# 1adrianb/binary-networks-pytorch

Hardware: AMD Instinct MI355X
Metric: images/sec binary ResNet-18 224x224 forward (higher is better)
Workload: dtype int1 xnor-popcount on the integer ALU (19 binary convs: two bit planes, v_bitop3_b32 + v_bcnt_u32_b32, int32 accumulation) + fp32 epilogues (alpha, BN, residual) + stem conv with fp32 operands split into fp16 hi+lo on v_mfma_f32_16x16x32_f16, fp32 accumulation (3e-7 relative; not IEEE fp32 — the exa

## Files before the change

binary-networks-pytorch_amd/bnn_amd/fastpath.py:

```python
from __future__ import annotations

import os
import threading
import warnings
import weakref
from dataclasses import dataclass
from typing import Optional

import torch
import torch.nn as nn

from . import hipops, native

_stats_lock = threading.Lock()
_stats = {"conv2d": 0, "conv1d": 0, "linear": 0, "weight_packs": 0, "conv2d_train": 0, "cell_op": 0, "cell": 0,
          "cell_op_train": 0, "reduce_train": 0, "linear_train": 0, "conv2d_real": 0, "conv2d_real_train": 0,
          "linear_real": 0, "linear_real_train": 0, "fconv": 0}

REAL_WEIGHTS = os.environ.get("BNN_AMD_REAL_WEIGHTS", "0") == "1"

MFMA_CONV = os.environ.get("BNN_AMD_MFMA_CONV", "1")
MFMA_CONV_SHAPES = {
    (128, 128, 28, 1, False): ((51.9, 37.8), (58.6, 45.2)),
    (128, 256, 28, 2, False): ((30.3, 26.2),),
    (256, 256, 14, 1, False): ((54.9, 33.4), (56.9, 38.9)),
    (256, 512, 14, 2, False): ((33.6, 23.8),),
    (512, 512, 7, 1, False): ((60.6, 32.0), (63.3, 39.2)),
}


def mfma_conv_admitted(C: int, O: int, H: int, stride: int, fold: bool) -> bool:
    if MFMA_CONV == "0":
        return False
    return MFMA_CONV == "all" or (C, O, H, stride, fold) in MFMA_CONV_SHAPES


MFMA_FOLD = os.environ.get("BNN_AMD_MFMA_FOLD", "1")
MFMA_FOLD_SHAPES = {
    (128, 128, 28, 64): (71.0, 61.2),
    (256, 256, 14, 128): (66.0, 50.3),
    (512, 512, 7, 256): (71.8, 45.3),
}


def mfma_fold_admitted(C: int, O: int, H: int, sc_C: int) -> bool:
    if MFMA_CONV == "0" or MFMA_FOLD == "0":
        return False
    return MFMA_FOLD == "all" or (C, O, H, sc_C) in MFMA_FOLD_SHAPES


FCONV_DECLINED_SHAPES = {
}


def fconv_admitted(C: int, H: int, W: int, stride: int) -> bool:
    return (C, H, W, stride) not in FCONV_DECLINED_SHAPES


def stats() -> dict:
    with _stats_lock:
        return dict(_stats)


def _bump(key: str) -> None:
    with _stats_lock:
        _stats[key] += 1


def strict_weights() -> bool:
    return os.environ.get("BNN_AMD_STRICT_WEIGHTS", "0") == "1"


@dataclass
class Plan:
    center: bool
    compute_alpha: bool
    scale: Optional[torch.Tensor]
    ste: bool = True


@dataclass
class RealPlan:
    scale: Optional[torch.Tensor]
    ste: bool = True


_HOOK_MODULES = ("bnn_amd.ops", "bnn_amd.bconfig", "bnn.ops", "bnn.bconfig")


def _is(obj, name: str) -> bool:
    t = type(obj)
    return t.__name__ == name and t.__module__ in _HOOK_MODULES


def _input_hook(pre) -> Optional[bool]:
    if _is(pre, "BasicInputBinarizer"):
        return True
    advanced = (_is(pre, "AdvancedInputBinarizer") and getattr(pre, "derivative_funct", None) is torch.tanh
                and isinstance(getattr(pre, "t", None), (int, float)) and pre.t > 0)
    return False if advanced else None


def _post_scale(post, out_channels: int):
    if _is(post, "Identity"):
        return True, None
    if _is(post, "BasicScaleBinarizer") and post.alpha.numel() == out_channels \
            and post.alpha.dim() >= 2 and post.alpha.shape[1] == out_channels:
        return True, post.alpha
    return False, None


def _recognise(layer: nn.Module, out_channels: int) -> Optional[Plan]:
    wpre = layer.weight_pre_process
    basic = _input_hook(layer.activation_pre_process)
    if basic is None or not _is(wpre, "XNORWeightBinarizer"):
        return None
    ok, scale = _post_scale(layer.activation_post_process, out_channels)
    if not ok:
        return None
    return Plan(bool(wpre.center_weights), bool(wpre.compute_alpha), scale, ste=basic)


def _recognise_real(layer: nn.Module, out_channels: int) -> Optional[RealPlan]:
    wpre = layer.weight_pre_process
    basic = _input_hook(layer.activation_pre_process)
    if basic is None:
        return None
    if not (type(wpre) is nn.Identity or _is(wpre, "Identity")) or wpre._forward_hooks or wpre._forward_pre_hooks:
        return None
    ok, scale = _post_scale(layer.activation_post_process, out_channels)
    if not ok:
        return None
    return RealPlan(scale, ste=basic)


def _eligible(layer: nn.Module, x: torch.Tensor, plan: Plan) -> bool:
    w = layer.weight
    if not (x.is_cuda and w.is_cuda and x.device == w.device):
        return False
    if x.dtype != w.dtype or x.dtype not in (torch.float32, torch.float16):
        return False
    if torch.is_grad_enabled():
        needs = x.requires_grad or w.requires_grad
        needs = needs or (layer.bias is not None and layer.bias.requires_grad)
        needs = needs or (plan.scale is not None and plan.scale.requires_grad)
        if needs:
            return False
    return True


def _eligible_train(layer: nn.Module, x: torch.Tensor) -> bool:
    from . import training
    w = layer.weight
    return (training.ENABLED and torch.is_grad_enabled() and x.is_cuda and w.is_cuda and x.device == w.device
            and x.dtype == torch.float32 and w.dtype == torch.float32)


def _numeric_padding(layer) -> bool:
    return not isinstance(layer.padding, str) and layer.padding_mode == "zeros" and layer.groups == 1


def _grouped_numeric_padding(layer) -> bool:
    return not isinstance(layer.padding, str) and layer.padding_mode == "zeros" and layer.groups > 1


def plan_conv2d(layer, x: torch.Tensor) -> Optional[Plan]:
    if x.dim() != 4 or not (_numeric_padding(layer) or _grouped_numeric_padding(layer)):
        return None
    plan = _recognise(layer, layer.out_channels)
    return plan if plan is not None and _eligible(layer, x, plan) else None


def plan_conv2d_train(layer, x: torch.Tensor) -> Optional[Plan]:
    from . import training
    if x.dim() != 4 or not (_numeric_padding(layer) or (training.GROUPED and _grouped_numeric_padding(layer))):
        return None
    plan = _recognise(layer, layer.out_channels)
    return plan if plan is not None and plan.ste and _eligible_train(layer, x) else None


def _real_applies(layer, x: torch.Tensor) -> Optional[RealPlan]:
    if not REAL_WEIGHTS or x.dim() != 4 or not _numeric_padding(layer) or torch.is_autocast_enabled():
        return None
    if x.dtype != torch.float32 or layer.weight.dtype != torch.float32:
        return None
    plan = _recognise_real(layer, layer.out_channels)
    if plan is None or not hipops.sconv_supported(x.shape, layer.weight.shape, layer.stride, layer.padding, layer.dilation):
        return None
    return plan


def plan_conv2d_real(layer, x: torch.Tensor) -> Optional[RealPlan]:
    plan = _real_applies(layer, x)
    return plan if plan is not None and _eligible(layer, x, plan) else None


def plan_conv2d_real_train(layer, x: torch.Tensor) -> Optional[RealPlan]:
    plan = _real_applies(layer, x)
    return plan if plan is not None and plan.ste and _eligible_train(layer, x) else None


def _real_linear_applies(layer, x: torch.Tensor) -> Optional[RealPlan]:
    if not REAL_WEIGHTS or x.dim() < 1 or torch.is_autocast_enabled():
        return None
    if x.dtype != torch.float32 or layer.weight.dtype != torch.float32:
        return None
    return _recognise_real(layer, layer.out_features)


def plan_linear_real(layer, x: torch.Tensor) -> Optional[RealPlan]:
    plan = _real_linear_applies(layer, x)
    return plan if plan is not None and _eligible(layer, x, plan) else None


def plan_linear_real_train(layer, x: torch.Tensor) -> Optional[RealPlan]:
    plan = _real_linear_applies(layer, x)
    return plan if plan is not None and plan.ste and _eligible_train(layer, x) else None


def plan_conv1d(layer, x: torch.Tensor) -> Optional[Plan]:
    if x.dim() != 3 or not (_numeric_padding(layer) or _grouped_numeric_padding(layer)):
        return None
    plan = _recognise(layer, layer.out_channels)
    return plan if plan is not None and _eligible(layer, x, plan) else None


def plan_linear(layer, x: torch.Tensor) -> Optional[Plan]:
    if x.dim() < 1:
        return None
    plan = _recognise(layer, layer.out_features)
    return plan if plan is not None and _eligible(layer, x, plan) else None


def plan_linear_train(layer, x: torch.Tensor) -> Optional[Plan]:
    from . import training
    if not training.LINEAR or x.dim() < 1 or torch.is_autocast_enabled():
        return None
    plan = _recognise(layer, layer.out_features)
    if plan is None or not plan.ste or not _eligible_train(layer, x):
        return None
    return plan if training._no_hooks(layer.weight_pre_process, backward=False) else None


def packed_weight(layer, plan: Plan, sync: bool = True, fresh: bool = False) -> hipops.PackedWeight:
    if strict_weights():
        sync, fresh = True, True
    master = layer.__dict__.get("_bnn_master")
    if master is not None:
        return _replica_packed_weight(layer, master, plan, fresh)
    w = layer.weight
    groups = getattr(layer, "groups", 1)
    key = (w.data_ptr(), w._version, str(w.device), tuple(w.shape), plan.center, plan.compute_alpha, groups)
    cached = layer.__dict__.get("_bnn_packed")
    sync = sync or cached is None
    if cached is not None and cached[1].zero_probe is not None and (sync or fresh or cached[0] != key):
        pw = cached[1]
        if pw.zero_found_later():
            layer.__dict__["_bnn_zero_seen"] = True
            warnings.warn("bnn_amd: a binary weight is exactly 0 (sign(0) == 0); a forward that ran before this "
                          "was known treated it as -1.  This layer now takes the zero-aware kernels.",
                          RuntimeWarning)
            cached = None
        else:
            pw.zero_probe = None
    if cached is not None and cached[0] == key and not fresh:
        return cached[1]
    sync = sync or layer.__dict__.get("_bnn_zero_seen", False)
    pw = _pack(w, plan, groups, sync)
    if pw.has_zero:
        layer.__dict__["_bnn_zero_seen"] = True
    layer.__dict__["_bnn_packed"] = (key, pw)
    _bump("weight_packs")
    return pw


def _pack(w: torch.Tensor, plan: Plan, groups: int, sync: bool) -> hipops.PackedWeight:
    if groups != 1:
        return hipops.pack_weight_grouped(w, groups, plan.center, plan.compute_alpha, sync=sync)
    return hipops.pack_weight(w, plan.center, plan.compute_alpha, sync=sync)


def _replica_packed_weight(layer, master, plan: Plan, fresh: bool = False) -> hipops.PackedWeight:
    mw = master.weight
    w = layer.weight
    groups = getattr(layer, "groups", 1)
    key = (mw.data_ptr(), mw._version, tuple(mw.shape), plan.center, plan.compute_alpha, groups)
    cache = master.__dict__.setdefault("_bnn_packed_replicas", {})
    dev = str(w.device)
    hit = cache.get(dev)
    if hit is not None and hit[0] == key and not fresh:
        return hit[1]
    pw = _pack(w, plan, groups, sync=True)
    cache[dev] = (key, pw)
    _bump("weight_packs")
    return pw


BLOCK_KEY, OP_KEY, CELL_KEY = TIER_KEYS = ("_bnn_auto_block", "_bnn_auto_op", "_bnn_auto_cell")


WATCH_KEY = "_bnn_watchers"


class _Watchers:

    def __init__(self) -> None:
        self.refs = weakref.WeakSet()

    def __deepcopy__(self, memo) -> "_Watchers":
        return _Watchers()

    def __reduce__(self):
        return (_Watchers, ())


def watch(model: nn.Module, executor) -> None:
    model.__dict__.setdefault(WATCH_KEY, _Watchers()).refs.add(executor)


def drop_executor(m: nn.Module) -> None:
    for key in TIER_KEYS:
        m.__dict__.pop(key, None)


def invalidate(module: nn.Module, executors: bool = True) -> int:
    n = 0
    for m in module.modules():
        if m.__dict__.pop("_bnn_packed", None) is not None:
            n += 1
        if m.__dict__.pop(REAL_KEY, None) is not None:
            n += 1
        m.__dict__.pop("_bnn_packed_replicas", None)
        if executors:
            drop_executor(m)
            for ex in tuple(getattr(m.__dict__.get(WATCH_KEY), "refs", ())):
                ex.mark_stale()
    from .tails import drop_derived
    drop_derived(module)
    return n


def _f32(t: Optional[torch.Tensor]) -> Optional[torch.Tensor]:
    return t if t is None or t.dtype == torch.float32 else t.detach().float()


def conv2d(layer, x: torch.Tensor, plan: Plan) -> torch.Tensor:
    native.require()
    pw = packed_weight(layer, plan)
    if layer.groups != 1:
        out = hipops.bconv2d_grouped(hipops.pack_act(x), pw, _f32(layer.bias), _f32(plan.scale), layer.stride,
                                     layer.padding, layer.dilation)
        _bump("conv2d")
        return out.to(x.dtype)
    out = hipops.bconv2d_direct(x, pw, _f32(layer.bias), _f32(plan.scale), layer.stride, layer.padding,
                                layer.dilation)
    _bump("conv2d")
    return out.to(x.dtype)


def conv2d_train(layer, x: torch.Tensor, plan: Plan) -> torch.Tensor:
    from . import training
    native.require()
    out = training.conv2d_train(layer, x, plan, packed_weight(layer, plan, sync=False, fresh=True))
    _bump("conv2d_train")
    return out


REAL_KEY = "_bnn_packed_real"


def real_packed_weight(layer) -> hipops.SconvWeight:
    w = layer.weight
    key = (w.data_ptr(), w._version, str(w.device), tuple(w.shape), "sconv")
    cached = layer.__dict__.get(REAL_KEY)
    if cached is not None and cached[0] == key and not strict_weights():
        return cached[1]
    pw = hipops.slinear_pack_weight(w) if w.dim() == 2 else hipops.sconv_pack_weight(w)
    layer.__dict__[REAL_KEY] = (key, pw)
    _bump("weight_packs")
    return pw


def conv2d_real(layer, x: torch.Tensor, plan: RealPlan) -> torch.Tensor:
    native.require()
    out = hipops.sconv2d(x, real_packed_weight(layer), layer.bias, plan.scale, layer.stride, layer.padding)
    _bump("conv2d_real")
    return out


def conv2d_real_train(layer, x: torch.Tensor, plan: RealPlan) -> torch.Tensor:
    from . import training
    native.require()
    out = training.sconv2d_train(layer, x, plan)
    _bump("conv2d_real_train")
    return out


def linear_real(layer, x: torch.Tensor, plan: RealPlan) -> torch.Tensor:
    native.require()
    scale = None if plan.scale is None else plan.scale.reshape(-1)
    out = hipops.slinear(x, real_packed_weight(layer), layer.bias, scale)
    _bump("linear_real")
    return out


def linear_real_train(layer, x: torch.Tensor, plan: RealPlan) -> torch.Tensor:
    from . import training
    native.require()
    out = training.slinear_train(layer, x, plan)
    _bump("linear_real_train")
    return out


def conv1d(layer, x: torch.Tensor, plan: Plan) -> torch.Tensor:
    native.require()
    pw = packed_weight(layer, plan)
    if layer.groups != 1:
        out = hipops.bconv2d_grouped(hipops.pack_act(x.unsqueeze(2)), pw, _f32(layer.bias), _f32(plan.scale),
                                     (1, layer.stride[0]), (0, layer.padding[0]), (1, layer.dilation[0]))
        _bump("conv1d")
        return out.squeeze(2).to(x.dtype)
    out = hipops.bconv2d_direct(x.unsqueeze(2), pw, _f32(layer.bias), _f32(plan.scale), (1, layer.stride[0]),
                                (0, layer.padding[0]), (1, layer.dilation[0]))
    _bump("conv1d")
    return out.squeeze(2).to(x.dtype)


def linear(layer, x: torch.Tensor, plan: Plan) -> torch.Tensor:
    native.require()
    pw = packed_weight(layer, plan)
    out = hipops.linear(x, pw, _f32(layer.bias), _f32(plan.scale))
    _bump("linear")
    return out.to(x.dtype)


def linear_train(layer, x: torch.Tensor, plan: Plan) -> torch.Tensor:
    from . import training
    native.require()
    out = training.linear_train(layer, x, plan, packed_weight(layer, plan, sync=False, fresh=True))
    _bump("linear_train")
    return out
```

binary-networks-pytorch_amd/csrc/bconv_mfma.hip:

```cpp
#include "bconv_core.h"

namespace bnn {

namespace {

using i32x4 = __attribute__((ext_vector_type(4))) int;

constexpr int kMfmaThreads = 256;
constexpr int kAccStride = 68;
constexpr int kAccBytes = 4 * 32 * kAccStride * 4;
constexpr int kMaxLds = 64 * 1024;
constexpr int kPatchSlots = 4;
constexpr int kParkStride = 72;
constexpr int kParkBytes = 4 * 64 * kParkStride * 2;
constexpr int kMaxLdsFold = 80 * 1024;

struct MfmaGeo {
  int tp;
  int groups;
  int ihw;
  int patch_cap;
  int nn;
  int n_in;
  uint32_t m_ihw;
  int s_ihw;
  int park_off;
};

struct ShortcutArgs8 {
  const uint32_t* P;
  const int8_t* W8;
  const float* alpha;
  const float* a;
  const float* b;
};

__device__ __forceinline__ uint32_t spread4(uint32_t word, int sh) {
  return __umul24((word >> sh) & 15u, 0x00204081u) & 0x01010101u;
}
__device__ __forceinline__ uint32_t expand4(uint32_t pw, uint32_t mw, int sh, bool nn) {
  const uint32_t p = spread4(pw, sh);
  if (nn) return p;
  return p | (spread4(mw, sh) * 0xFFu);
}

__device__ __forceinline__ int centre_of(const Geo& g, const MfmaGeo& mg, int q, int* oy, int* ox) {
  const int hw = g.Ho * g.Wo;
  const int n = (int)fast_div((uint32_t)q, g.m_hw, g.s_hw);
  const int r = q - n * hw;
  *oy = (int)fast_div((uint32_t)r, g.m_wo, g.s_wo);
  *ox = r - *oy * g.Wo;
  return n * mg.ihw + *oy * g.sh * g.Wd + *ox * g.sw;
}

template <int EP, bool DS = false>
__global__ __launch_bounds__(kMfmaThreads) void bconv_mfma_kernel(const uint32_t* __restrict__ P,
                                                                  const uint32_t* __restrict__ M,
                                                                  const int8_t* __restrict__ W8, BNN_EPI_PARAMS,
                                                                  const Geo g, const MfmaGeo mg,
                                                                  const uint32_t* __restrict__ dsP,
                                                                  const int8_t* __restrict__ dsW8,
                                                                  const float* __restrict__ ds_alpha,
                                                                  const float* __restrict__ ds_a,
                                                                  const float* __restrict__ ds_b) {
  static_assert(!DS || EP == EP_OUT, "the fold belongs to BN + residual + ReLU -> fp32 + planes");
  BNN_EPI_INIT;
  [[maybe_unused]] const ShortcutArgs8 sc{dsP, dsW8, ds_alpha, ds_a, ds_b};
  extern __shared__ __attribute__((aligned(16))) unsigned char lds[];
  const int tid = threadIdx.x, lane = tid & 63;
  const int wave = __builtin_amdgcn_readfirstlane(tid >> 6);
  const int lrow = lane & 15, lgrp = lane >> 4;
  const int pwaves = mg.tp >> 6;
  const int wave_pix = (wave % pwaves) * 64;
  const int wave_ch = (wave / pwaves) * 64;
  const int q0 = blockIdx.x * mg.tp;
  const int o_wave = blockIdx.y * (64 * (4 / pwaves)) + wave_ch;

  int ty, tx;
  const int c_first = centre_of(g, mg, q0, &ty, &tx);
  const int c_last = centre_of(g, mg, min(q0 + mg.tp, g.npix) - 1, &ty, &tx);
  const int l_lo = max(c_first - g.Wd - 1, 0);
  const int patch_len = min(min(c_last + g.Wd + 1, mg.n_in - 1) - l_lo + 1, mg.patch_cap);
  const int zero_idx = mg.patch_cap;

  int base[4];
  uint32_t okm[4];
#pragma unroll
  for (int pt = 0; pt < 4; ++pt) {
    const int q = min(q0 + wave_pix + 16 * pt + lrow, g.npix - 1);
    int oy, ox;
    base[pt] = centre_of(g, mg, q, &oy, &ox) - l_lo;
    uint32_t m = 0u;
#pragma unroll
    for (int t = 0; t < 9; ++t) {
      const int iy = oy * g.sh - 1 + t / 3, ix = ox * g.sw - 1 + t % 3;
      const bool ok = (unsigned)iy < (unsigned)g.H && (unsigned)ix < (unsigned)g.Wd;
      m |= (ok ? 1u : 0u) << t;
    }
    okm[pt] = m;
  }

  i32x4 acc[4][4];
#pragma unroll
  for (int ct = 0; ct < 4; ++ct)
#pragma unroll
    for (int pt = 0; pt < 4; ++pt) acc[ct][pt] = i32x4{0, 0, 0, 0};

  if (tid < 4) reinterpret_cast<uint4*>(lds + (size_t)zero_idx * 64)[tid] = uint4{0u, 0u, 0u, 0u};

  const bool nn = mg.nn != 0;
  const uint2* P2 = reinterpret_cast<const uint2*>(P);
  const uint2* M2 = reinterpret_cast<const uint2*>(M);
  const int8_t* wbase = W8 + (size_t)(o_wave >> 6) * mg.groups * (9 * 4096) + lane * 16;

  const int ksteps = mg.groups * 9;
  auto a_load = [&](i32x4 (&dst)[4], int k) {
    const int8_t* src = wbase + (size_t)min(k, ksteps - 1) * 4096;
#pragma unroll
    for (int ct = 0; ct < 4; ++ct) dst[ct] = *reinterpret_cast<const i32x4*>(src + ct * 1024);
  };
  auto b_frag = [&](int pt, int t) -> i32x4 {
    const int off = (t / 3 - 1) * g.Wd + (t % 3 - 1);
    const int idx = ((okm[pt] >> t) & 1u) ? min(base[pt] + off, zero_idx) : zero_idx;
    return *reinterpret_cast<const i32x4*>(lds + (size_t)idx * 64 + lgrp * 16);
  };
  unsigned wi0[kPatchSlots];
  uint2 pv[kPatchSlots], mv[kPatchSlots];
#pragma unroll
  for (int sl = 0; sl < kPatchSlots; ++sl) {
    const int L = l_lo + min(tid + sl * kMfmaThreads, patch_len - 1);
    const int n = (int)fast_div((uint32_t)L, mg.m_ihw, mg.s_ihw);
    wi0[sl] = (unsigned)(n * mg.groups * mg.ihw + (L - n * mg.ihw));
    pv[sl] = uint2{0u, 0u};
    mv[sl] = uint2{0u, 0u};
  }
  auto request = [&](int gi) {
#pragma unroll
    for (int sl = 0; sl < kPatchSlots; ++sl)
      if (sl * kMfmaThreads < patch_len) {
        pv[sl] = P2[wi0[sl] + (unsigned)(gi * mg.ihw)];
        if (!nn) mv[sl] = M2[wi0[sl] + (unsigned)(gi * mg.ihw)];
      }
  };
  auto expand = [&]() {
#pragma unroll
    for (int sl = 0; sl < kPatchSlots; ++sl) {
      const int i = tid + sl * kMfmaThreads;
      if (i < patch_len) {
        uint4* dst = reinterpret_cast<uint4*>(lds + (size_t)i * 64);
#pragma unroll
        for (int h = 0; h < 4; ++h) {
          const uint32_t pw = h < 2 ? pv[sl].x : pv[sl].y, mw = h < 2 ? mv[sl].x : mv[sl].y;
          const int s0 = 16 * (h & 1);
          dst[h] = uint4{expand4(pw, mw, s0, nn), expand4(pw, mw, s0 + 4, nn), expand4(pw, mw, s0 + 8, nn),
                         expand4(pw, mw, s0 + 12, nn)};
        }
      }
    }
  };

  request(0);
  i32x4 a_buf[3][4];
  if constexpr (DS) {
    const int sg = g.ds_cw >> 1;
    uint2 scw[4];
    {
      const int q = min(q0 + tid, g.npix - 1), hw = g.Ho * g.Wo;
      const int n = (int)fast_div((uint32_t)q, g.m_hw, g.s_hw), r = q - n * hw;
      const int oy = (int)fast_div((uint32_t)r, g.m_wo, g.s_wo), ox = r - oy * g.Wo;
      const uint2* S2 = reinterpret_cast<const uint2*>(sc.P);
      if (g.ds_w > 0) {
        const unsigned shw = (unsigned)(g.ds_h * g.ds_w);
        const int y0 = 2 * oy, x0 = 2 * ox;
        const bool x1 = x0 + 1 < g.ds_w, y1 = y0 + 1 < g.ds_h;
        const unsigned b0 = (unsigned)n * (unsigned)sg * shw + (unsigned)(y0 * g.ds_w + x0);
        static_for<4>([&](auto GI) {
          constexpr int gi = GI;
          uint2 v{0u, 0u};
          if (gi < sg) {
            const unsigned b = b0 + (unsigned)gi * shw;
            v = S2[b];
            const uint2 a = S2[x1 ? b + 1 : b], c = S2[y1 ? b + (unsigned)g.ds_w : b],
                        e = S2[(x1 && y1) ? b + (unsigned)g.ds_w + 1 : b];
            v.x |= a.x | c.x | e.x;
            v.y |= a.y | c.y | e.y;
          }
          scw[gi] = v;
        });
      } else {
        const unsigned b0 = (unsigned)n * (unsigned)sg * (unsigned)hw + (unsigned)r;
        static_for<4>([&](auto GI) {
          constexpr int gi = GI;
          scw[gi] = gi < sg ? S2[b0 + (unsigned)(gi * hw)] : uint2{0u, 0u};
        });
      }
    }
    const int8_t* sbase = sc.W8 + (size_t)(o_wave >> 6) * sg * 4096 + lane * 16;
    auto sa_load = [&](i32x4 (&dst)[4], int k) {
      const int8_t* src = sbase + (size_t)min(k, sg - 1) * 4096;
#pragma unroll
      for (int ct = 0; ct < 4; ++ct) dst[ct] = *reinterpret_cast<const i32x4*>(src + ct * 1024);
    };
    sa_load(a_buf[0], 0);
    sa_load(a_buf[1], 1);
    static_for<4>([&](auto K) {
      constexpr int k = K;
      if (k < sg) {
        if (k > 0) __syncthreads();
        if (tid < mg.tp) {
          uint4* dst = reinterpret_cast<uint4*>(lds + (size_t)tid * 64);
#pragma unroll
          for (int h = 0; h < 4; ++h) {
            const uint32_t pw = h < 2 ? scw[k].x : scw[k].y;
            const int s0 = 16 * (h & 1);
            dst[h] = uint4{expand4(pw, 0u, s0, true), expand4(pw, 0u, s0 + 4, true), expand4(pw, 0u, s0 + 8, true),
                           expand4(pw, 0u, s0 + 12, true)};
          }
        }
        __syncthreads();
        sa_load(a_buf[(k + 2) % 3], k + 2);
        i32x4 b_sc[4];
#pragma unroll
        for (int pt = 0; pt < 4; ++pt)
          b_sc[pt] = *reinterpret_cast<const i32x4*>(lds + (size_t)(wave_pix + 16 * pt + lrow) * 64 + lgrp * 16);
        __builtin_amdgcn_sched_barrier(0);
#pragma unroll
        for (int ct = 0; ct < 4; ++ct)
#pragma unroll
          for (int pt = 0; pt < 4; ++pt)
            acc[ct][pt] = __builtin_amdgcn_mfma_i32_16x16x64_i8(a_buf[k % 3][ct], b_sc[pt], acc[ct][pt], 0, 0, 0);
        __builtin_amdgcn_sched_barrier(0);
      }
    });
  }
  a_load(a_buf[0], 0);
  a_load(a_buf[1], 1);
  if constexpr (DS) {
    short* park = reinterpret_cast<short*>(lds + mg.park_off) + wave * (64 * kParkStride);
#pragma unroll
    for (int ct = 0; ct < 4; ++ct)
#pragma unroll
      for (int pt = 0; pt < 4; ++pt) {
        const i32x4 v = acc[ct][pt];
        *reinterpret_cast<uint2*>(park + (16 * pt + lrow) * kParkStride + 16 * ct + 4 * lgrp) =
            uint2{((uint32_t)v[0] & 0xFFFFu) | ((uint32_t)v[1] << 16), ((uint32_t)v[2] & 0xFFFFu) | ((uint32_t)v[3] << 16)};
        acc[ct][pt] = i32x4{0, 0, 0, 0};
      }
  }
#pragma unroll 1
  for (int gi = 0; gi < mg.groups; ++gi) {
    __syncthreads();
    expand();
    __syncthreads();
    if (gi + 1 < mg.groups) request(gi + 1);
    i32x4 b_cur[4];
#pragma unroll
    for (int pt = 0; pt < 4; ++pt) b_cur[pt] = b_frag(pt, 0);
#pragma unroll
    for (int t = 0; t < 9; ++t) {
      i32x4 b_nxt[4];
      a_load(a_buf[(t + 2) % 3], gi * 9 + t + 2);
      if (t < 8) {
#pragma unroll
        for (int pt = 0; pt < 4; ++pt) b_nxt[pt] = b_frag(pt, t + 1);
      }
      __builtin_amdgcn_sched_barrier(0);
#pragma unroll
      for (int ct = 0; ct < 4; ++ct)
#pragma unroll
        for (int pt = 0; pt < 4; ++pt)
          acc[ct][pt] = __builtin_amdgcn_mfma_i32_16x16x64_i8(a_buf[t % 3][ct], b_cur[pt], acc[ct][pt], 0, 0, 0);
      __builtin_amdgcn_sched_barrier(0);
      if (t < 8) {
#pragma unroll
        for (int pt = 0; pt < 4; ++pt) b_cur[pt] = b_nxt[pt];
      }
    }
  }

  const Pix px = decode_pixel<true>(g, q0 + wave_pix + lane);
  int* tbuf = reinterpret_cast<int*>(lds) + wave * (32 * kAccStride);
#pragma unroll
  for (int h = 0; h < 2; ++h) {
    const int o0 = o_wave + 32 * h;
    float resv[32];
    if constexpr (DS) {
      using f2 = __attribute__((ext_vector_type(2))) float;
      const uint4* pr = reinterpret_cast<const uint4*>(reinterpret_cast<const short*>(lds + mg.park_off) +
                                                       wave * (64 * kParkStride) + lane * kParkStride + 32 * h);
      uint32_t w[16];
#pragma unroll
      for (int i = 0; i < 4; ++i) {
        const uint4 v = pr[i];
        w[4 * i] = v.x; w[4 * i + 1] = v.y; w[4 * i + 2] = v.z; w[4 * i + 3] = v.w;
      }
#pragma unroll
      for (int j = 0; j < 32; j += 2) {
        const int o = o0 + j;
        const f2 d = f2{(float)((int)(w[j >> 1] << 16) >> 16), (float)((int)w[j >> 1] >> 16)};
        const f2 t = __builtin_elementwise_fma(f2{sc.alpha[o], sc.alpha[o + 1]}, d, f2{0.0f, 0.0f});
        const f2 r = __builtin_elementwise_fma(t, f2{sc.a[o], sc.a[o + 1]}, f2{sc.b[o], sc.b[o + 1]});
        resv[j] = r.x;
        resv[j + 1] = r.y;
      }
    } else {
      prefetch_residual<32, EP, true>(g, px, o0, epi, resv);
    }
    __syncthreads();
#pragma unroll
    for (int c2 = 0; c2 < 2; ++c2)
#pragma unroll
      for (int pt = 0; pt < 4; ++pt)
#pragma unroll
        for (int r = 0; r < 4; ++r)
          tbuf[(16 * c2 + 4 * lgrp + r) * kAccStride + 16 * pt + lrow] = acc[2 * h + c2][pt][r];
    __syncthreads();
    int dot[32];
#pragma unroll
    for (int j = 0; j < 32; ++j) dot[j] = tbuf[j * kAccStride + lane];
    uint32_t pbits = 0u, mbits = 0u;
    epilogue<32, EP, true>(g, px, o0, dot, resv, epi, pbits, mbits, 0, 1.0f, 0.0f);
    uint32_t xorw = 0u;
    if constexpr (EP == EP_MIDT) xorw = (uint32_t)epi.thr[kThrStride * o0 + 1];
    store_packed(g, px, o0 >> 5, pbits, mbits, epi, true, xorw);
  }
}

__global__ __launch_bounds__(256) void pack_weight_i8_kernel(const uint32_t* __restrict__ wbits,
                                                             const uint32_t* __restrict__ wnz, int O, int taps,
                                                             int cw32, int cwc, uint32_t* __restrict__ w8) {
  const int groups = cw32 >> 1, nchunk = cw32 / cwc, per_o = taps * cwc;
  const size_t total = (size_t)O * groups * taps * 16;
  const size_t d = (size_t)blockIdx.x * 256 + threadIdx.x;
  if (d >= total) return;
  const int e4 = (int)(d & 3), lane = (int)((d >> 2) & 63), ct = (int)((d >> 8) & 3);
  size_t rest = d >> 10;
  const int t = (int)(rest % taps);
  rest /= taps;
  const int gi = (int)(rest % groups), ob64 = (int)(rest / groups);
  const int o = 64 * ob64 + 16 * ct + (lane & 15);
  const int c0 = 64 * gi + 16 * (lane >> 4) + 4 * e4;
  const int cw_abs = c0 >> 5, ch = cw_abs / cwc, cw = cw_abs - ch * cwc;
  const size_t wi = ((size_t)((o >> 5) * nchunk + ch) * kOCB + (o & 31)) * per_o + t * cwc + cw;
  const uint32_t b = wbits[wi] >> (c0 & 31), z = wnz ? wnz[wi] >> (c0 & 31) : 15u;
  uint32_t v = 0u;
#pragma unroll
  for (int k = 0; k < 4; ++k) {
    const uint32_t byte = ((z >> k) & 1u) ? (((b >> k) & 1u) ? 0x01u : 0xFFu) : 0u;
    v |= byte << (8 * k);
  }
  w8[d] = v;
}

long long centre_span(const ConvP& p, int tp) {
  const long long s = p.sw, k = tp - 1, hw = (long long)p.Ho * p.Wo;
  const long long row_extra = (long long)p.sh * p.Wd - (long long)p.Wo * s;
  const long long img_extra = (long long)p.H * p.Wd - (long long)p.Ho * p.sh * p.Wd;
  return k * s + (k + p.Wo - 1) / p.Wo * (row_extra > 0 ? row_extra : 0) + (k + hw - 1) / hw * (img_extra > 0 ? img_extra : 0);
}

size_t lds_bytes_of(int patch_cap) {
  const size_t patch = (size_t)(patch_cap + 1) * 64;
  return patch > (size_t)kAccBytes ? patch : (size_t)kAccBytes;
}

int choose_tile(const ConvP& p, int* patch_cap, size_t park = 0) {
  const size_t lds_max = park ? (size_t)kMaxLdsFold : (size_t)kMaxLds;
  const int order[2] = {(p.O % 128 == 0 && p.C >= 128) ? 128 : 256, (p.O % 128 == 0 && p.C >= 128) ? 256 : 128};
  for (int tp : order) {
    if (tp == 128 && p.O % 128 != 0) continue;
    const long long cap = centre_span(p, tp) + 2LL * p.Wd + 3;
    if (cap <= kPatchSlots * kMfmaThreads && lds_bytes_of((int)cap) + park <= lds_max) {
      *patch_cap = (int)cap;
      return tp;
    }
  }
  return 0;
}

template <int EP>
void launch_ep(const ConvP& p, const Geo& g, const MfmaGeo& mg, const void* w8, dim3 grid, size_t ldsb, hipStream_t s) {
  hipLaunchKernelGGL((bconv_mfma_kernel<EP>), grid, dim3(kMfmaThreads), ldsb, s, p.P, p.M,
                     static_cast<const int8_t*>(w8), BNN_EPI_ACTUALS, g, mg, static_cast<const uint32_t*>(nullptr),
                     static_cast<const int8_t*>(nullptr), static_cast<const float*>(nullptr),
                     static_cast<const float*>(nullptr), static_cast<const float*>(nullptr));
}

}

size_t weight_i8_bytes(int O, int C, int KH, int KW) {
  if (O <= 0 || C <= 0 || KH != 3 || KW != 3 || O % 64 != 0 || C % 64 != 0) return 0;
  return (size_t)O * (size_t)C * 9;
}

int launch_pack_weight_i8(const uint32_t* wbits, const uint32_t* wnz, const bnn_hip_wlayout& L, int O, void* w8,
                          hipStream_t s) {
  const size_t dwords = (size_t)O * (L.cw32 >> 1) * L.taps * 16;
  hipLaunchKernelGGL(pack_weight_i8_kernel, dim3((unsigned)((dwords + 255) / 256)), dim3(256), 0, s, wbits, wnz, O, L.taps,
                     L.cw32, L.cwc, static_cast<uint32_t*>(w8));
  return hipGetLastError() == hipSuccess ? BNN_HIP_OK : BNN_HIP_ERR_LAUNCH;
}

size_t shortcut_weight_i8_bytes(int O, int C) {
  if (O <= 0 || O % 64 != 0 || (C != 64 && C != 128 && C != 256)) return 0;
  return (size_t)O * (size_t)C;
}

int launch_pack_shortcut_weight_i8(const uint32_t* wbits, int O, int C, void* w8, hipStream_t s) {
  const int cw32 = C / 32;
  const size_t dwords = (size_t)O * (cw32 >> 1) * 16;
  hipLaunchKernelGGL(pack_weight_i8_kernel, dim3((unsigned)((dwords + 255) / 256)), dim3(256), 0, s, wbits,
                     static_cast<const uint32_t*>(nullptr), O, 1, cw32, cw32, static_cast<uint32_t*>(w8));
  return hipGetLastError() == hipSuccess ? BNN_HIP_OK : BNN_HIP_ERR_LAUNCH;
}

namespace {
bool mfma_dense_rule(const ConvP& p, int flags, size_t park) {
  if (flags & BNN_HIP_FLAG_FORCE_GENERIC) return false;
  if (p.KH != 3 || p.KW != 3 || p.ph != 1 || p.pw != 1 || p.dh != 1 || p.dw != 1) return false;
  if (p.sh != p.sw || (p.sh != 1 && p.sh != 2)) return false;
  if (p.C % 64 != 0 || p.O % 64 != 0 || !small_indices(p)) return false;
  if (p.raw || p.prelu || p.pack_a || p.pack_b || p.eflags != 0) return false;
  if (p.c_off != 0 || p.c_tot != p.O) return false;
  if ((long long)p.N * p.H * p.Wd >= (1ll << 30)) return false;
  int cap = 0;
  return choose_tile(p, &cap, park) != 0;
}
}

bool mfma_conv_applies(const ConvP& p, int flags) { return !p.ds_P && mfma_dense_rule(p, flags, 0); }

bool mfma_fold_applies(const ConvP& p, int flags) {
  if (!p.ds_P || p.res || p.thr) return false;
  if (!(flags & BNN_HIP_FLAG_ACT_NONNEG) || (flags & BNN_HIP_FLAG_WEIGHT_ZEROS)) return false;
  if (shortcut_weight_i8_bytes(p.O, p.ds_C) == 0) return false;
  if (make_geo(p).flags != kFlagsOut) return false;
  return mfma_dense_rule(p, flags, (size_t)kParkBytes);
}

namespace {
MfmaGeo make_mfma_geo(const ConvP& p, int flags, int tp, int cap) {
  MfmaGeo mg;
  mg.tp = tp;
  mg.groups = p.C / 64;
  mg.ihw = p.H * p.Wd;
  mg.patch_cap = cap;
  mg.nn = (flags & BNN_HIP_FLAG_ACT_NONNEG) ? 1 : 0;
  mg.n_in = p.N * p.H * p.Wd;
  div_magic((uint32_t)mg.ihw, mg.m_ihw, mg.s_ihw);
  mg.park_off = (int)lds_bytes_of(cap);
  return mg;
}
}

int launch_bconv_mfma_fold(const ConvP& p, int flags, const void* w8, const void* sc_w8, hipStream_t s) {
  int cap = 0;
  const int tp = choose_tile(p, &cap, (size_t)kParkBytes);
  if (!mfma_fold_applies(p, flags) || tp == 0) return BNN_HIP_ERR_UNSUPPORTED;
  const Geo g = make_geo(p);
  const MfmaGeo mg = make_mfma_geo(p, flags, tp, cap);
  const dim3 grid((unsigned)((p.npix + tp - 1) / tp), (unsigned)(p.O / (tp == 256 ? 64 : 128)));
  const size_t ldsb = lds_bytes_of(cap) + (size_t)kParkBytes;
  auto kern = bconv_mfma_kernel<EP_OUT, true>;
  if (hipFuncSetAttribute(reinterpret_cast<const void*>(kern), hipFuncAttributeMaxDynamicSharedMemorySize,
                          kMaxDynamicLds) != hipSuccess)
    return BNN_HIP_ERR_LAUNCH;
  hipLaunchKernelGGL(kern, grid, dim3(kMfmaThreads), ldsb, s, p.P, p.M, static_cast<const int8_t*>(w8), BNN_EPI_ACTUALS, g,
                     mg, p.ds_P, static_cast<const int8_t*>(sc_w8), p.ds_alpha, p.ds_a, p.ds_b);
  return hipGetLastError() == hipSuccess ? BNN_HIP_OK : BNN_HIP_ERR_LAUNCH;
}

int launch_bconv_mfma(const ConvP& p, int flags, const void* w8, hipStream_t s) {
  int cap = 0;
  const int tp = choose_tile(p, &cap);
  if (!mfma_conv_applies(p, flags) || tp == 0) return BNN_HIP_ERR_UNSUPPORTED;
  const Geo g = make_geo(p);
  const MfmaGeo mg = make_mfma_geo(p, flags, tp, cap);
  const dim3 grid((unsigned)((p.npix + tp - 1) / tp), (unsigned)(p.O / (tp == 256 ? 64 : 128)));
  const size_t ldsb = lds_bytes_of(cap);
  const int f = g.flags;
  const bool fused = (f & (EF_BN | EF_RES | EF_RELU | EF_PACK)) != 0;
  if (f == kFlagsMid && p.thr) launch_ep<EP_MIDT>(p, g, mg, w8, grid, ldsb, s);
  else if (f == kFlagsMid) launch_ep<EP_MID>(p, g, mg, w8, grid, ldsb, s);
  else if (f == kFlagsOut) launch_ep<EP_OUT>(p, g, mg, w8, grid, ldsb, s);
  else if (f == kFlagsOutP) launch_ep<EP_OUTP>(p, g, mg, w8, grid, ldsb, s);
  else if (f == kFlagsLast) launch_ep<EP_LAST>(p, g, mg, w8, grid, ldsb, s);
  else if (fused) launch_ep<EP_RUNTIME>(p, g, mg, w8, grid, ldsb, s);
  else launch_ep<EP_PLAIN>(p, g, mg, w8, grid, ldsb, s);
  return hipGetLastError() == hipSuccess ? BNN_HIP_OK : BNN_HIP_ERR_LAUNCH;
}

}
```

Before: 328,000.

## Reshape MFMA binary conv wave tile to 128 pixels by 32 channels with padded LDS planes

Each wave now covers 128 pixels by 32 output channels instead of 64 by 64. The LDS patch is stored as four separate 16-byte planes, and a virtual zero row is inserted between image rows. Border handling uses precomputed left, centre and right addresses plus a far address clamped to a zero slot, which replaces the per-tap validity mask and index clamp. The aim is to cut LDS address arithmetic and bank conflicts and to change A/B fragment reuse, at the cost of more B fragment loads per wave, more registers, and a larger patch span.

Result: no change. 328,800 (median of 3 runs) (+0.3%).

```diff
diff --git a/binary-networks-pytorch_amd/bnn_amd/fastpath.py b/binary-networks-pytorch_amd/bnn_amd/fastpath.py
--- a/binary-networks-pytorch_amd/bnn_amd/fastpath.py
+++ b/binary-networks-pytorch_amd/bnn_amd/fastpath.py
@@ -21,11 +21,11 @@
 
 MFMA_CONV = os.environ.get("BNN_AMD_MFMA_CONV", "1")
 MFMA_CONV_SHAPES = {
-    (128, 128, 28, 1, False): ((51.9, 37.8), (58.6, 45.2)),
-    (128, 256, 28, 2, False): ((30.3, 26.2),),
-    (256, 256, 14, 1, False): ((54.9, 33.4), (56.9, 38.9)),
-    (256, 512, 14, 2, False): ((33.6, 23.8),),
-    (512, 512, 7, 1, False): ((60.6, 32.0), (63.3, 39.2)),
+    (128, 128, 28, 1, False): ((51.9, 38.0), (58.6, 47.8)),
+    (128, 256, 28, 2, False): ((30.3, 27.8),),
+    (256, 256, 14, 1, False): ((54.9, 34.3), (56.9, 39.7)),
+    (256, 512, 14, 2, False): ((33.6, 23.6),),
+    (512, 512, 7, 1, False): ((60.6, 32.2), (63.3, 41.4)),
 }
 
 
@@ -37,9 +37,9 @@
 
 MFMA_FOLD = os.environ.get("BNN_AMD_MFMA_FOLD", "1")
 MFMA_FOLD_SHAPES = {
-    (128, 128, 28, 64): (71.0, 61.2),
-    (256, 256, 14, 128): (66.0, 50.3),
-    (512, 512, 7, 256): (71.8, 45.3),
+    (128, 128, 28, 64): (71.0, 60.8),
+    (256, 256, 14, 128): (66.0, 47.5),
+    (512, 512, 7, 256): (71.8, 44.8),
 }
 
 
diff --git a/binary-networks-pytorch_amd/csrc/bconv_mfma.hip b/binary-networks-pytorch_amd/csrc/bconv_mfma.hip
--- a/binary-networks-pytorch_amd/csrc/bconv_mfma.hip
+++ b/binary-networks-pytorch_amd/csrc/bconv_mfma.hip
@@ -11,8 +11,11 @@
 constexpr int kAccBytes = 4 * 32 * kAccStride * 4;
 constexpr int kMaxLds = 64 * 1024;
 constexpr int kPatchSlots = 4;
-constexpr int kParkStride = 72;
-constexpr int kParkBytes = 4 * 64 * kParkStride * 2;
+constexpr int kWavePix = 128;
+constexpr int kWaveCh = 32;
+constexpr uint32_t kFarAddr = 0x40000000u;
+constexpr int kParkStride = 36;
+constexpr int kParkBytes = 4 * kWavePix * kParkStride * 2;
 constexpr int kMaxLdsFold = 80 * 1024;
 
 struct MfmaGeo {
@@ -20,10 +23,14 @@
   int groups;
   int ihw;
   int patch_cap;
+  int plane;
   int nn;
-  int n_in;
-  uint32_t m_ihw;
-  int s_ihw;
+  int hp;
+  int n_pad;
+  uint32_t m_w;
+  int s_w;
+  uint32_t m_hp;
+  int s_hp;
   int park_off;
 };
 
@@ -50,7 +57,7 @@
   const int r = q - n * hw;
   *oy = (int)fast_div((uint32_t)r, g.m_wo, g.s_wo);
   *ox = r - *oy * g.Wo;
-  return n * mg.ihw + *oy * g.sh * g.Wd + *ox * g.sw;
+  return (n * mg.hp + *oy * g.sh + 1) * g.Wd + *ox * g.sw;
 }
 
 template <int EP, bool DS = false>
@@ -70,74 +77,73 @@
   const int tid = threadIdx.x, lane = tid & 63;
   const int wave = __builtin_amdgcn_readfirstlane(tid >> 6);
   const int lrow = lane & 15, lgrp = lane >> 4;
-  const int pwaves = mg.tp >> 6;
-  const int wave_pix = (wave % pwaves) * 64;
-  const int wave_ch = (wave / pwaves) * 64;
+  const int pwaves = mg.tp >> 7;
+  const int wave_pix = (wave % pwaves) * kWavePix;
+  const int wave_ch = (wave / pwaves) * kWaveCh;
   const int q0 = blockIdx.x * mg.tp;
-  const int o_wave = blockIdx.y * (64 * (4 / pwaves)) + wave_ch;
+  const int o_wave = blockIdx.y * (kWaveCh * (4 / pwaves)) + wave_ch;
 
   int ty, tx;
   const int c_first = centre_of(g, mg, q0, &ty, &tx);
   const int c_last = centre_of(g, mg, min(q0 + mg.tp, g.npix) - 1, &ty, &tx);
   const int l_lo = max(c_first - g.Wd - 1, 0);
-  const int patch_len = min(min(c_last + g.Wd + 1, mg.n_in - 1) - l_lo + 1, mg.patch_cap);
-  const int zero_idx = mg.patch_cap;
-
-  int base[4];
-  uint32_t okm[4];
-#pragma unroll
-  for (int pt = 0; pt < 4; ++pt) {
+  const int patch_len = min(min(c_last + g.Wd + 1, mg.n_pad - 1) - l_lo + 1, mg.patch_cap);
+  const uint32_t zero_addr = (uint32_t)(3 * mg.plane + mg.patch_cap * 16);
+
+  uint32_t ad_c[8], ad_l[8], ad_r[8];
+#pragma unroll
+  for (int pt = 0; pt < 8; ++pt) {
     const int q = min(q0 + wave_pix + 16 * pt + lrow, g.npix - 1);
     int oy, ox;
-    base[pt] = centre_of(g, mg, q, &oy, &ox) - l_lo;
-    uint32_t m = 0u;
-#pragma unroll
-    for (int t = 0; t < 9; ++t) {
-      const int iy = oy * g.sh - 1 + t / 3, ix = ox * g.sw - 1 + t % 3;
-      const bool ok = (unsigned)iy < (unsigned)g.H && (unsigned)ix < (unsigned)g.Wd;
-      m |= (ok ? 1u : 0u) << t;
-    }
-    okm[pt] = m;
-  }
-
-  i32x4 acc[4][4];
-#pragma unroll
-  for (int ct = 0; ct < 4; ++ct)
-#pragma unroll
-    for (int pt = 0; pt < 4; ++pt) acc[ct][pt] = i32x4{0, 0, 0, 0};
-
-  if (tid < 4) reinterpret_cast<uint4*>(lds + (size_t)zero_idx * 64)[tid] = uint4{0u, 0u, 0u, 0u};
+    const int base = centre_of(g, mg, q, &oy, &ox) - l_lo;
+    const int ix = ox * g.sw;
+    ad_c[pt] = (uint32_t)(base * 16 + lgrp * mg.plane);
+    ad_l[pt] = ix >= 1 ? ad_c[pt] - 16u : kFarAddr;
+    ad_r[pt] = ix + 1 < g.Wd ? ad_c[pt] + 16u : kFarAddr;
+  }
+  const int row_bytes = g.Wd * 16;
+
+  i32x4 acc[2][8];
+#pragma unroll
+  for (int ct = 0; ct < 2; ++ct)
+#pragma unroll
+    for (int pt = 0; pt < 8; ++pt) acc[ct][pt] = i32x4{0, 0, 0, 0};
+
+  if (tid == 0) *reinterpret_cast<uint4*>(lds + zero_addr) = uint4{0u, 0u, 0u, 0u};
 
   const bool nn = mg.nn != 0;
   const uint2* P2 = reinterpret_cast<const uint2*>(P);
   const uint2* M2 = reinterpret_cast<const uint2*>(M);
-  const int8_t* wbase = W8 + (size_t)(o_wave >> 6) * mg.groups * (9 * 4096) + lane * 16;
+  const int8_t* wbase = W8 + (size_t)(o_wave >> 6) * mg.groups * (9 * 4096) + ((o_wave & 63) >> 4) * 1024 + lane * 16;
 
   const int ksteps = mg.groups * 9;
-  auto a_load = [&](i32x4 (&dst)[4], int k) {
+  auto a_load = [&](i32x4 (&dst)[2], int k) {
     const int8_t* src = wbase + (size_t)min(k, ksteps - 1) * 4096;
 #pragma unroll
-    for (int ct = 0; ct < 4; ++ct) dst[ct] = *reinterpret_cast<const i32x4*>(src + ct * 1024);
+    for (int ct = 0; ct < 2; ++ct) dst[ct] = *reinterpret_cast<const i32x4*>(src + ct * 1024);
   };
   auto b_frag = [&](int pt, int t) -> i32x4 {
-    const int off = (t / 3 - 1) * g.Wd + (t % 3 - 1);
-    const int idx = ((okm[pt] >> t) & 1u) ? min(base[pt] + off, zero_idx) : zero_idx;
-    return *reinterpret_cast<const i32x4*>(lds + (size_t)idx * 64 + lgrp * 16);
+    const int dy = t / 3 - 1, dx = t % 3 - 1;
+    const uint32_t off = (uint32_t)(dy * row_bytes);
+    const uint32_t addr = dx == 0 ? ad_c[pt] + off : min((dx < 0 ? ad_l[pt] : ad_r[pt]) + off, zero_addr);
+    return *reinterpret_cast<const i32x4*>(lds + addr);
   };
+  constexpr unsigned kZeroRow = 0xFFFFFFFFu;
   unsigned wi0[kPatchSlots];
   uint2 pv[kPatchSlots], mv[kPatchSlots];
 #pragma unroll
   for (int sl = 0; sl < kPatchSlots; ++sl) {
     const int L = l_lo + min(tid + sl * kMfmaThreads, patch_len - 1);
-    const int n = (int)fast_div((uint32_t)L, mg.m_ihw, mg.s_ihw);
-    wi0[sl] = (unsigned)(n * mg.groups * mg.ihw + (L - n * mg.ihw));
+    const int row = (int)fast_div((uint32_t)L, mg.m_w, mg.s_w), x = L - row * g.Wd;
+    const int n = (int)fast_div((uint32_t)row, mg.m_hp, mg.s_hp), yy = row - n * mg.hp;
+    wi0[sl] = yy == 0 ? kZeroRow : (unsigned)(n * mg.groups * mg.ihw + (yy - 1) * g.Wd + x);
     pv[sl] = uint2{0u, 0u};
     mv[sl] = uint2{0u, 0u};
   }
   auto request = [&](int gi) {
 #pragma unroll
     for (int sl = 0; sl < kPatchSlots; ++sl)
-      if (sl * kMfmaThreads < patch_len) {
+      if (sl * kMfmaThreads < patch_len && wi0[sl] != kZeroRow) {
         pv[sl] = P2[wi0[sl] + (unsigned)(gi * mg.ihw)];
         if (!nn) mv[sl] = M2[wi0[sl] + (unsigned)(gi * mg.ihw)];
       }
@@ -147,20 +153,20 @@
     for (int sl = 0; sl < kPatchSlots; ++sl) {
       const int i = tid + sl * kMfmaThreads;
       if (i < patch_len) {
-        uint4* dst = reinterpret_cast<uint4*>(lds + (size_t)i * 64);
 #pragma unroll
         for (int h = 0; h < 4; ++h) {
           const uint32_t pw = h < 2 ? pv[sl].x : pv[sl].y, mw = h < 2 ? mv[sl].x : mv[sl].y;
           const int s0 = 16 * (h & 1);
-          dst[h] = uint4{expand4(pw, mw, s0, nn), expand4(pw, mw, s0 + 4, nn), expand4(pw, mw, s0 + 8, nn),
-                         expand4(pw, mw, s0 + 12, nn)};
+          *reinterpret_cast<uint4*>(lds + h * mg.plane + i * 16) =
+              uint4{expand4(pw, mw, s0, nn), expand4(pw, mw, s0 + 4, nn), expand4(pw, mw, s0 + 8, nn),
+                    expand4(pw, mw, s0 + 12, nn)};
         }
       }
     }
   };
 
   request(0);
-  i32x4 a_buf[3][4];
+  i32x4 a_buf[3][2];
   if constexpr (DS) {
     const int sg = g.ds_cw >> 1;
     uint2 scw[4];
@@ -195,11 +201,11 @@
         });
       }
     }
-    const int8_t* sbase = sc.W8 + (size_t)(o_wave >> 6) * sg * 4096 + lane * 16;
-    auto sa_load = [&](i32x4 (&dst)[4], int k) {
+    const int8_t* sbase = sc.W8 + (size_t)(o_wave >> 6) * sg * 4096 + ((o_wave & 63) >> 4) * 1024 + lane * 16;
+    auto sa_load = [&](i32x4 (&dst)[2], int k) {
       const int8_t* src = sbase + (size_t)min(k, sg - 1) * 4096;
 #pragma unroll
-      for (int ct = 0; ct < 4; ++ct) dst[ct] = *reinterpret_cast<const i32x4*>(src + ct * 1024);
+      for (int ct = 0; ct < 2; ++ct) dst[ct] = *reinterpret_cast<const i32x4*>(src + ct * 1024);
     };
     sa_load(a_buf[0], 0);
     sa_load(a_buf[1], 1);
@@ -208,26 +214,26 @@
       if (k < sg) {
         if (k > 0) __syncthreads();
         if (tid < mg.tp) {
-          uint4* dst = reinterpret_cast<uint4*>(lds + (size_t)tid * 64);
 #pragma unroll
           for (int h = 0; h < 4; ++h) {
             const uint32_t pw = h < 2 ? scw[k].x : scw[k].y;
             const int s0 = 16 * (h & 1);
-            dst[h] = uint4{expand4(pw, 0u, s0, true), expand4(pw, 0u, s0 + 4, true), expand4(pw, 0u, s0 + 8, true),
-                           expand4(pw, 0u, s0 + 12, true)};
+            *reinterpret_cast<uint4*>(lds + h * mg.plane + tid * 16) =
+                uint4{expand4(pw, 0u, s0, true), expand4(pw, 0u, s0 + 4, true), expand4(pw, 0u, s0 + 8, true),
+                      expand4(pw, 0u, s0 + 12, true)};
           }
         }
         __syncthreads();
         sa_load(a_buf[(k + 2) % 3], k + 2);
-        i32x4 b_sc[4];
-#pragma unroll
-        for (int pt = 0; pt < 4; ++pt)
-          b_sc[pt] = *reinterpret_cast<const i32x4*>(lds + (size_t)(wave_pix + 16 * pt + lrow) * 64 + lgrp * 16);
+        i32x4 b_sc[8];
+#pragma unroll
+        for (int pt = 0; pt < 8; ++pt)
+          b_sc[pt] = *reinterpret_cast<const i32x4*>(lds + lgrp * mg.plane + (wave_pix + 16 * pt + lrow) * 16);
         __builtin_amdgcn_sched_barrier(0);
 #pragma unroll
-        for (int ct = 0; ct < 4; ++ct)
-#pragma unroll
-          for (int pt = 0; pt < 4; ++pt)
+        for (int ct = 0; ct < 2; ++ct)
+#pragma unroll
+          for (int pt = 0; pt < 8; ++pt)
             acc[ct][pt] = __builtin_amdgcn_mfma_i32_16x16x64_i8(a_buf[k % 3][ct], b_sc[pt], acc[ct][pt], 0, 0, 0);
         __builtin_amdgcn_sched_barrier(0);
       }
@@ -236,11 +242,11 @@
   a_load(a_buf[0], 0);
   a_load(a_buf[1], 1);
   if constexpr (DS) {
-    short* park = reinterpret_cast<short*>(lds + mg.park_off) + wave * (64 * kParkStride);
-#pragma unroll
-    for (int ct = 0; ct < 4; ++ct)
-#pragma unroll
-      for (int pt = 0; pt < 4; ++pt) {
+    short* park = reinterpret_cast<short*>(lds + mg.park_off) + wave * (kWavePix * kParkStride);
+#pragma unroll
+    for (int ct = 0; ct < 2; ++ct)
+#pragma unroll
+      for (int pt = 0; pt < 8; ++pt) {
         const i32x4 v = acc[ct][pt];
         *reinterpret_cast<uint2*>(park + (16 * pt + lrow) * kParkStride + 16 * ct + 4 * lgrp) =
             uint2{((uint32_t)v[0] & 0xFFFFu) | ((uint32_t)v[1] << 16), ((uint32_t)v[2] & 0xFFFFu) | ((uint32_t)v[3] << 16)};
@@ -253,46 +259,46 @@
     expand();
     __syncthreads();
     if (gi + 1 < mg.groups) request(gi + 1);
-    i32x4 b_cur[4];
-#pragma unroll
-    for (int pt = 0; pt < 4; ++pt) b_cur[pt] = b_frag(pt, 0);
+    i32x4 b_cur[8];
+#pragma unroll
+    for (int pt = 0; pt < 8; ++pt) b_cur[pt] = b_frag(pt, 0);
 #pragma unroll
     for (int t = 0; t < 9; ++t) {
-      i32x4 b_nxt[4];
+      i32x4 b_nxt[8];
       a_load(a_buf[(t + 2) % 3], gi * 9 + t + 2);
       if (t < 8) {
 #pragma unroll
-        for (int pt = 0; pt < 4; ++pt) b_nxt[pt] = b_frag(pt, t + 1);
+        for (int pt = 0; pt < 8; ++pt) b_nxt[pt] = b_frag(pt, t + 1);
       }
       __builtin_amdgcn_sched_barrier(0);
 #pragma unroll
-      for (int ct = 0; ct < 4; ++ct)
-#pragma unroll
-        for (int pt = 0; pt < 4; ++pt)
+      for (int ct = 0; ct < 2; ++ct)
+#pragma unroll
+        for (int pt = 0; pt < 8; ++pt)
           acc[ct][pt] = __builtin_amdgcn_mfma_i32_16x16x64_i8(a_buf[t % 3][ct], b_cur[pt], acc[ct][pt], 0, 0, 0);
       __builtin_amdgcn_sched_barrier(0);
       if (t < 8) {
 #pragma unroll
-        for (int pt = 0; pt < 4; ++pt) b_cur[pt] = b_nxt[pt];
+        for (int pt = 0; pt < 8; ++pt) b_cur[pt] = b_nxt[pt];
       }
     }
   }
 
-  const Pix px = decode_pixel<true>(g, q0 + wave_pix + lane);
   int* tbuf = reinterpret_cast<int*>(lds) + wave * (32 * kAccStride);
+  const int o0 = o_wave;
 #pragma unroll
   for (int h = 0; h < 2; ++h) {
-    const int o0 = o_wave + 32 * h;
+    const Pix px = decode_pixel<true>(g, q0 + wave_pix + 64 * h + lane);
     float resv[32];
     if constexpr (DS) {
       using f2 = __attribute__((ext_vector_type(2))) float;
-      const uint4* pr = reinterpret_cast<const uint4*>(reinterpret_cast<const short*>(lds + mg.park_off) +
-                                                       wave * (64 * kParkStride) + lane * kParkStride + 32 * h);
+      const uint2* pr = reinterpret_cast<const uint2*>(reinterpret_cast<const short*>(lds + mg.park_off) +
+                                                       wave * (kWavePix * kParkStride) + (64 * h + lane) * kParkStride);
       uint32_t w[16];
 #pragma unroll
-      for (int i = 0; i < 4; ++i) {
-        const uint4 v = pr[i];
-        w[4 * i] = v.x; w[4 * i + 1] = v.y; w[4 * i + 2] = v.z; w[4 * i + 3] = v.w;
+      for (int i = 0; i < 8; ++i) {
+        const uint2 v = pr[i];
+        w[2 * i] = v.x; w[2 * i + 1] = v.y;
       }
 #pragma unroll
       for (int j = 0; j < 32; j += 2) {
@@ -308,12 +314,12 @@
     }
     __syncthreads();
 #pragma unroll
-    for (int c2 = 0; c2 < 2; ++c2)
+    for (int ct = 0; ct < 2; ++ct)
 #pragma unroll
       for (int pt = 0; pt < 4; ++pt)
 #pragma unroll
         for (int r = 0; r < 4; ++r)
-          tbuf[(16 * c2 + 4 * lgrp + r) * kAccStride + 16 * pt + lrow] = acc[2 * h + c2][pt][r];
+          tbuf[(16 * ct + 4 * lgrp + r) * kAccStride + 16 * pt + lrow] = acc[ct][4 * h + pt][r];
     __syncthreads();
     int dot[32];
 #pragma unroll
@@ -325,6 +331,7 @@
     store_packed(g, px, o0 >> 5, pbits, mbits, epi, true, xorw);
   }
 }
+
 
 __global__ __launch_bounds__(256) void pack_weight_i8_kernel(const uint32_t* __restrict__ wbits,
                                                              const uint32_t* __restrict__ wnz, int O, int taps,
@@ -355,12 +362,15 @@
 long long centre_span(const ConvP& p, int tp) {
   const long long s = p.sw, k = tp - 1, hw = (long long)p.Ho * p.Wo;
   const long long row_extra = (long long)p.sh * p.Wd - (long long)p.Wo * s;
-  const long long img_extra = (long long)p.H * p.Wd - (long long)p.Ho * p.sh * p.Wd;
-  return k * s + (k + p.Wo - 1) / p.Wo * (row_extra > 0 ? row_extra : 0) + (k + hw - 1) / hw * (img_extra > 0 ? img_extra : 0);
-}
+  const long long img_extra = (long long)(p.H + 1) * p.Wd - (long long)p.Ho * p.sh * p.Wd;
+  const long long imgs = (k + hw - 1) / hw < p.N - 1 ? (k + hw - 1) / hw : p.N - 1;
+  return k * s + (k + p.Wo - 1) / p.Wo * (row_extra > 0 ? row_extra : 0) + imgs * (img_extra > 0 ? img_extra : 0);
+}
+
+size_t plane_bytes_of(int patch_cap) { return ((size_t)(patch_cap + 1) * 16 + 255) & ~(size_t)255; }
 
 size_t lds_bytes_of(int patch_cap) {
-  const size_t patch = (size_t)(patch_cap + 1) * 64;
+  const size_t patch = 4 * plane_bytes_of(patch_cap);
   return patch > (size_t)kAccBytes ? patch : (size_t)kAccBytes;
 }
 
@@ -422,7 +432,7 @@
   if (p.C % 64 != 0 || p.O % 64 != 0 || !small_indices(p)) return false;
   if (p.raw || p.prelu || p.pack_a || p.pack_b || p.eflags != 0) return false;
   if (p.c_off != 0 || p.c_tot != p.O) return false;
-  if ((long long)p.N * p.H * p.Wd >= (1ll << 30)) return false;
+  if (((long long)p.N * (p.H + 1) + 1) * p.Wd >= (1ll << 30)) return false;
   int cap = 0;
   return choose_tile(p, &cap, park) != 0;
 }
@@ -445,9 +455,12 @@
   mg.groups = p.C / 64;
   mg.ihw = p.H * p.Wd;
   mg.patch_cap = cap;
+  mg.plane = (int)plane_bytes_of(cap);
   mg.nn = (flags & BNN_HIP_FLAG_ACT_NONNEG) ? 1 : 0;
-  mg.n_in = p.N * p.H * p.Wd;
-  div_magic((uint32_t)mg.ihw, mg.m_ihw, mg.s_ihw);
+  mg.hp = p.H + 1;
+  mg.n_pad = (p.N * mg.hp + 1) * p.Wd;
+  div_magic((uint32_t)p.Wd, mg.m_w, mg.s_w);
+  div_magic((uint32_t)mg.hp, mg.m_hp, mg.s_hp);
   mg.park_off = (int)lds_bytes_of(cap);
   return mg;
 }
```
